# mitenjain/nanopore

Hardware: AMD Instinct MI355X
Metric: DP cells/sec (banded pair-HMM realign: forward + backward + posterior per cell) (higher is better)
Workload: dtype f32

## Files before the change

### nanopore_amd/csrc/npr_device.h

```cpp
#pragma once
#include <cstdint>

#include "npr_internal.h"
#include "npr_band.h"

namespace npr {

struct Task {
    int64_t x_off;
    int64_t y_off;
    int64_t band_off;
    int64_t pair_off;
    int32_t lX, lY;
    int32_t D;
    int32_t pair_cap;
    int32_t flags;
    int32_t model;
    int32_t xs, ys;
    int32_t read;
    int32_t cells_pad;
    int64_t ctl_off;
    int64_t tile_off;
    int64_t rowmask_off;
};

struct Stripe {
    int32_t X;
    int32_t K;
    int32_t df, dl;
    uint32_t row0;
    int32_t pad[3];
};

struct TaskOut {
    float tot_m;
    int32_t tot_e;
    float btot_m;
    int32_t btot_e;
    int32_t npairs;
    int32_t status;
};

struct KernelArgs {
    const Task *tasks;
    TaskOut *outs;
    int32_t *queue;
    int32_t ntasks;
    const DevModel *models;
    const uint8_t *seq;
    const int32_t *lo;
    const int32_t *n;
    const uint32_t *coff;
    const Stripe *stripes;
    const uint32_t *rowmask;
    unsigned long long *prof;
    const int64_t *region;
    const uint32_t *ctl;
    char *F;
    int64_t slot_stride;
    int32_t slot_base;
    int32_t *px;
    int32_t *py;
    float *pp;
    float threshold;
    int32_t wcap;
    float *Bv;
    int32_t *Be;
    float *ring;
    float *Fx;
    double *em_T;
    double *em_E;
};

constexpr int EM_BINS = 32;

struct CompactArgs {
    const Task *tasks;
    const TaskOut *outs;
    const int64_t *dst_off;
    int32_t ntasks;
    const int32_t *px;
    const int32_t *py;
    const float *pp;
    int32_t *cx;
    int32_t *cy;
    float *cp;
};

int launch_generic(const KernelArgs &a, int grid, int threads, size_t lds_bytes, bool dense, bool global_ring, void *stream);
int launch_em(const KernelArgs &a, int grid, size_t lds_bytes, bool global_ring, void *stream);
size_t em_extra_lds_bytes();
int launch_compact(const CompactArgs &a, void *stream);
int launch_stair(const KernelArgs &a, int R, int grid, void *stream);
int launch_wide(const KernelArgs &a, int R, int NW, int grid, void *stream);
int launch_em_stair(const KernelArgs &a, int R, int grid, void *stream);
size_t em_stair_lds_bytes();
struct MeaArgs {
    const Task *tasks;
    const TaskOut *outs;
    int32_t ntasks, n_reads;
    const int32_t *px, *py;
    const float *pp;
    const int64_t *rx_off;
    const int64_t *ry_off;
    const int64_t *rp_off;
    int32_t *cnt, *start, *colsum;
    int32_t *sx, *sy, *sq, *back;
    int32_t *kx, *ky, *kq, *kback;
    int4 *vrec;
    int32_t *kept;
    const int32_t *np, *poff, *pboff, *lane_read, *lane_piece;
    int32_t *pb, *pbest;
    int32_t n_pieces;
    int32_t *best_who;
    int32_t *read_flag;
    double gap_gamma, match_gamma;
    int32_t ring;
    const int32_t *order;
    const int32_t *read_first, *read_ntasks, *task_of;
    int32_t sort_lds_bytes;
    int32_t sort_threads;
    int32_t any_global_sort;
    const int64_t *cnt_off;
    int32_t ring_only;
    int32_t *ops_tmp;
    const int64_t *ot_off;
    int32_t *n_ops, *chain_len;
    int64_t *chain_mass;
    uint32_t *ops_dense;
    const int64_t *od_off;
    int32_t *max_run;
    uint16_t *ops_dense16;
};
int launch_tile(const KernelArgs &a, int R, int NW, int grid, void *stream, bool flat = false);
size_t tile_lds_bytes(int nw);
int64_t tile_scratch_cells(int64_t rows, int R);
struct PlanSeg {
    int64_t point_first;
    int64_t band_off;
    int32_t pieces, lX, lY, pad;
};
struct SegSummary {
    int64_t cells;
    int64_t generic_cells;
    int32_t max_width;
    int32_t bad;
    int32_t rough;
    int32_t pad;
};
constexpr int kSchedClasses = 7;
constexpr int kSchedR[kSchedClasses] = {1, 2, 4, 2, 2, 4, 4};
constexpr int kSchedNW[kSchedClasses] = {1, 1, 1, 4, 8, 8, 12};
struct PlanArgs {
    int32_t n_segs, fixed_mode, width;
    const PlanPoint *points;
    const PlanSeg *segs;
    int32_t *lo, *n;
    SegSummary *summary;
};
struct SchedArgs {
    int32_t n_segs;
    const PlanSeg *segs;
    const SegSummary *summary;
    const int32_t *lo, *n;
    const int64_t *ctl_off;
    const uint32_t *cand;
    uint32_t *ctl;
    int32_t *cls;
    int64_t *cells;
};
struct StripeArgs {
    int32_t count, R;
    const int32_t *seg_index;
    const PlanSeg *segs;
    const SegSummary *summary;
    const int32_t *lo, *n;
    const int64_t *tile_off;
    Stripe *stripes;
    int64_t *rows;
};
struct CoffArgs {
    int32_t n_segs;
    const PlanSeg *segs;
    const int32_t *n;
    uint32_t *coff;
};
int launch_plan_bands(const PlanArgs &a, void *stream);
template <int R>
NPR_HD constexpr uint32_t row_bias() { return R == 4 ? 2048u : 1024u; }
NPR_HD constexpr bool stair_fits(int64_t rows, int slots) { return rows * slots < (int64_t(1) << 29) - 512; }
struct RowMaskArgs {
    int32_t count;
    const int32_t *seg_index;
    const PlanSeg *segs;
    const int32_t *lo, *n;
    const int64_t *tile_off;
    const Stripe *stripes;
    const int64_t *mask_off;
    uint32_t *out;
};
int launch_plan_rowmask(const RowMaskArgs &a, void *stream);
size_t plan_sched_chunk_bytes(int64_t n_chunks);
int64_t plan_sched_chunks_of(int64_t D);
int launch_plan_sched(const SchedArgs &a, const int64_t *chunk_off, int64_t n_chunks, void *chunks, int32_t *cur, uint32_t cand_union, void *stream);
// ... 80 lines not shown
```

### nanopore_amd/csrc/npr_finish.cpp

```cpp
#include "npr_api_internal.h"

extern "C" {

}
namespace npr_impl {

int32_t fetch_pairs(npr_batch *b) {
    npr_ctx *ctx = b->ctx;
    if (b->pairs_ready) return NPR_OK;
    StageTimer tm("fetch_pairs");
    const int64_t ntasks = static_cast<int64_t>(b->tasks.size());
    const std::vector<int64_t> &dst = b->task_dst;
    const int32_t *hx = nullptr, *hy = nullptr;
    const float *hp = nullptr;
    const int64_t total = ntasks ? dst[ntasks] : 0;
    if (total) {
        DevBuf<int64_t> d_dst;
        DevBuf<int32_t> d_cx, d_cy;
        DevBuf<float> d_cp;
        hipError_t e;
        if ((e = d_dst.alloc_from(ctx, ntasks + 1)) != hipSuccess || (e = d_cx.alloc_from(ctx, total)) != hipSuccess ||
            (e = d_cy.alloc_from(ctx, total)) != hipSuccess || (e = d_cp.alloc_from(ctx, total)) != hipSuccess)
            return fail(ctx, NPR_ERR_NOMEM, "npr_batch_finish: hipMalloc", e);
        HIP_TRY(ctx, hipMemcpyAsync(d_dst.p, dst.data(), d_dst.bytes(), hipMemcpyHostToDevice, ctx->stream));
// ... 100 lines not shown
        if (b->read_status[i] != NPR_OK) return;
        int32_t *out = runs + 3 * run_off[i];
        int64_t x = 0, y = 0;
        for (int64_t q = b->guide_off[i]; q < b->guide_off[i + 1]; ++q) {
            const int32_t op = b->guide_ops[2 * q], len = b->guide_ops[2 * q + 1];
            if (op == NPR_OP_M) {
                if (len > 0) out[0] = static_cast<int32_t>(x), out[1] = static_cast<int32_t>(y), out[2] = len, out += 3;
                x += len, y += len;
            } else if (op == NPR_OP_I) {
                y += len;
            } else {
                x += len;
            }
        }
    });
    tm.lap("runs");
    DevBuf<int64_t> d_run_off;
    DevBuf<int32_t> d_runs;
    hipError_t e;
    if ((e = d_run_off.alloc_from(ctx, n + 1)) != hipSuccess || (e = b->d_rs_gx_off.alloc_from(ctx, n + 1)) != hipSuccess ||
        (e = d_runs.alloc_from(ctx, std::max<size_t>(3 * static_cast<size_t>(run_off[n]), 1))) != hipSuccess ||
        (e = b->d_rs_gy.alloc_from(ctx, std::max<int64_t>(gx_off[n], 1))) != hipSuccess)
        return fail(ctx, NPR_ERR_NOMEM, "npr_batch_create: hipMalloc (rescore tables)", e);
    HIP_TRY(ctx, hipMemcpyAsync(d_run_off.p, run_off.data(), sizeof(int64_t) * (n + 1), hipMemcpyHostToDevice, ctx->stream));
    HIP_TRY(ctx, hipMemcpyAsync(b->d_rs_gx_off.p, gx_off.data(), sizeof(int64_t) * (n + 1), hipMemcpyHostToDevice, ctx->stream));
    if (run_bytes) HIP_TRY(ctx, hipMemcpyAsync(d_runs.p, runs, run_bytes, hipMemcpyHostToDevice, ctx->stream));
    HIP_TRY(ctx, hipMemsetAsync(b->d_rs_gy.p, 0xff, sizeof(int32_t) * std::max<int64_t>(gx_off[n], 1), ctx->stream));
    RescoreArgs ra{static_cast<int32_t>(n), 0, d_run_off.p, d_runs.p, b->d_rs_gx_off.p, b->d_rs_gy.p, nullptr, nullptr, nullptr, nullptr, nullptr, nullptr, shift};
    const int rc = launch_rescore_table(ra, ctx->stream);
    if (rc != 0) return fail(ctx, NPR_ERR_HIP, "k_rescore_table launch", static_cast<hipError_t>(rc));
    HIP_TRY(ctx, hipStreamSynchronize(ctx->stream));
    tm.lap("table");
    b->rs_shift = shift, b->rs_staged = true;
    return NPR_OK;
}

int32_t rescore_sum(npr_batch *b, std::vector<double> &score) {
    npr_ctx *ctx = b->ctx;
    const int64_t n = b->n_reads, ntasks = static_cast<int64_t>(b->tasks.size());
    DevBuf<unsigned long long> d_sum;
    hipError_t e;
    if ((e = d_sum.alloc_from(ctx, n)) != hipSuccess) return fail(ctx, NPR_ERR_NOMEM, "npr_batch_finish: hipMalloc (rescore sums)", e);
    HIP_TRY(ctx, hipMemsetAsync(d_sum.p, 0, sizeof(unsigned long long) * n, ctx->stream));
    RescoreArgs ra{static_cast<int32_t>(n), static_cast<int32_t>(ntasks), nullptr, nullptr, b->d_rs_gx_off.p, b->d_rs_gy.p, b->d_tasks.p, b->d_outs.p,
                   b->d_px.p, b->d_py.p, b->d_pp.p, d_sum.p, b->rs_shift};
    const int rc = launch_rescore_sum(ra, ctx->stream);
    if (rc != 0) return fail(ctx, NPR_ERR_HIP, "k_rescore_sum launch", static_cast<hipError_t>(rc));
    std::vector<unsigned long long> sum(n);
    HIP_TRY(ctx, hipMemcpyAsync(sum.data(), d_sum.p, sizeof(unsigned long long) * n, hipMemcpyDeviceToHost, ctx->stream));
    HIP_TRY(ctx, hipStreamSynchronize(ctx->stream));
    score.assign(n, 0.0);
    for (int64_t i = 0; i < n; ++i)
        if (b->rs_columns[i] > 0) score[i] = std::ldexp(static_cast<double>(sum[i]), -b->rs_shift) / static_cast<double>(b->rs_columns[i]);
    return NPR_OK;
}

int32_t device_mea(npr_batch *b) {
    npr_ctx *ctx = b->ctx;
    std::unique_lock<std::mutex> arena_lock(ctx->arena->mu, std::defer_lock);
    if (!ctx->overlap) arena_lock.lock();
    ++ctx->arena->epoch;
    StageTimer tm("device_mea");
    const int64_t n = b->n_reads, ntasks = static_cast<int64_t>(b->tasks.size());
    std::vector<int64_t> rx(n + 1, 0), ry(n + 1, 0), rp(n + 1, 0), ot(n + 1, 0), od(n + 1, 0);
    for (int64_t i = 0; i < n; ++i) {
        const bool ok = b->results[i].status == NPR_OK;
        const int64_t lX = ok ? b->ref_len[i] : 0, lY = ok ? b->read_len[i] : 0, np = ok ? b->pair_off[i + 1] - b->pair_off[i] : 0;
        rx[i + 1] = rx[i] + lX + 1;
        ry[i + 1] = ry[i] + lY;
        rp[i + 1] = rp[i] + np;
        ot[i + 1] = ot[i] + 3 * std::min({np, lX, lY}) + 2;
    }
    const int ring = 8192;
    const int64_t total = rp[n];
    constexpr int64_t kMaxPieces = 64, kLanesWanted = 64 * 5 * 256;
    const int64_t kPiecePairs = std::min<int64_t>(2048, std::max<int64_t>(128, total / kLanesWanted));
    std::vector<int32_t> np(n);
    int64_t n_pieces = 0;
    for (int64_t i = 0; i < n; ++i) np[i] = static_cast<int32_t>(std::min(kMaxPieces, std::max<int64_t>(1, (rp[i + 1] - rp[i] + kPiecePairs - 1) / kPiecePairs))), n_pieces += np[i];
    if (!ctx->mea) ctx->mea = new MeaScratch;
    MeaScratch &m = *ctx->mea;
    hipError_t e;
    const int64_t lds_span = ctx->opt[NPR_OPT_MEA_GLOBAL_SORT] != 0 ? 0 : 16 * 1024;
    int64_t span = 0;
    std::vector<int64_t> cnt_off(n + 1, -1);
    int64_t cnt_total = 0;
    for (int64_t i = 0; i < n; ++i) {
        const int64_t sp = std::max(rx[i + 1] - rx[i], ry[i + 1] - ry[i]);
        if (sp <= lds_span) span = std::max(span, sp);
        else cnt_off[i] = cnt_total, cnt_total += rx[i + 1] - rx[i];
    }
    const bool sort_in_lds = cnt_total == 0;
    const size_t ntask_map = b->task_of.size();
    const size_t n_cnt = sort_in_lds ? 1 : static_cast<size_t>(cnt_total);
    {
        auto al = [](size_t bytes) { return (bytes + 255) & ~size_t(255); };
        const size_t need = al(8 * 5 * (n + 1)) + al(8 * n) + al(8 * (n + 1)) + 2 * al(4 * n_cnt) + al(4 * (ry[n] + 1)) + al(4 * (12 * total + 16)) +
                            al(4 * 6 * n) + al(4 * 2 * ot[n]) + al(4 * (3 * n + ntask_map)) + al(4 * ot[n]) + al(4 * (4 * n_pieces + 4 * n));
        const bool arena_fits = ctx->arena->F && need <= static_cast<size_t>(ctx->arena->cells.load()) * 8;
        bool in_arena = !ctx->overlap && arena_fits;
        for (;;) {
            char *cur = ctx->arena->F;
            if (in_arena && poison_byte() >= 0) {
                HIP_TRY(ctx, hipStreamSynchronize(ctx->stream));
                poison(ctx->arena->F, need);
            }
            auto take = [&](auto &buf, size_t count) -> hipError_t {
                using T = std::remove_pointer_t<decltype(buf.p)>;
                if (!in_arena) return buf.reserve(count);
                buf.borrow(reinterpret_cast<T *>(cur), count);
                cur += al(sizeof(T) * count);
                return hipSuccess;
            };
            if ((e = take(m.off, 5 * (n + 1))) == hipSuccess && (e = take(m.mass, n)) == hipSuccess && (e = take(m.od, n + 1)) == hipSuccess &&
                (e = take(m.cnt, n_cnt)) == hipSuccess && (e = take(m.start, n_cnt)) == hipSuccess && (e = take(m.col, ry[n] + 1)) == hipSuccess &&
                (e = take(m.sorted, 12 * total + 16)) == hipSuccess && (e = take(m.small, 6 * n)) == hipSuccess && (e = take(m.tmp, 2 * ot[n])) == hipSuccess &&
                (e = take(m.map, 3 * n + ntask_map)) == hipSuccess && (e = take(m.dense, ot[n])) == hipSuccess &&
                (e = take(m.pieces, 4 * n_pieces + 4 * n)) == hipSuccess)
                break;
            (void)hipGetLastError();
            if (!in_arena && ctx->overlap && arena_fits) {
                m.off.release(), m.mass.release(), m.od.release(), m.cnt.release(), m.start.release(), m.col.release(), m.sorted.release();
                m.small.release(), m.tmp.release(), m.map.release(), m.dense.release(), m.pieces.release();
                ctx->cache_flush();
                arena_lock.lock();
                if (!(ctx->arena->F && need <= static_cast<size_t>(ctx->arena->cells.load()) * 8)) return 1;
                ++ctx->arena->epoch;
                in_arena = true;
                continue;
            }
            return 1;
        }
    }
    HIP_TRY(ctx, hipMemcpyAsync(m.map.p, b->read_first_task.data(), sizeof(int32_t) * n, hipMemcpyHostToDevice, ctx->stream));
    HIP_TRY(ctx, hipMemcpyAsync(m.map.p + n, b->read_ntasks.data(), sizeof(int32_t) * n, hipMemcpyHostToDevice, ctx->stream));
    HIP_TRY(ctx, hipMemcpyAsync(m.map.p + 2 * n, b->task_of.data(), sizeof(int32_t) * ntask_map, hipMemcpyHostToDevice, ctx->stream));
    std::vector<int32_t> order(n);
    std::iota(order.begin(), order.end(), 0);
    std::stable_sort(order.begin(), order.end(), [&](int32_t x, int32_t y) { return rp[x + 1] - rp[x] > rp[y + 1] - rp[y]; });
    HIP_TRY(ctx, hipMemcpyAsync(m.map.p + 2 * n + ntask_map, order.data(), sizeof(int32_t) * n, hipMemcpyHostToDevice, ctx->stream));
    {
        std::vector<int32_t> tab(3 * n + 2 * n_pieces);
        int32_t *const t_np = tab.data(), *const t_poff = t_np + n, *const t_pboff = t_poff + n, *const t_lr = t_pboff + n, *const t_lp = t_lr + n_pieces;
        int64_t at = 0;
        for (int64_t k = 0; k < n; ++k) {
            const int32_t r = order[k];
            t_np[r] = np[r], t_poff[r] = static_cast<int32_t>(at), t_pboff[r] = static_cast<int32_t>(at + k);
            for (int32_t j = 0; j < np[r]; ++j) t_lr[at + j] = r, t_lp[at + j] = j;
            at += np[r];
        }
        HIP_TRY(ctx, hipMemcpyAsync(m.pieces.p, tab.data(), sizeof(int32_t) * tab.size(), hipMemcpyHostToDevice, ctx->stream));
    }
    std::vector<int64_t> offs(5 * (n + 1));
    std::copy(cnt_off.begin(), cnt_off.end(), offs.begin() + 4 * (n + 1));
    std::copy(rx.begin(), rx.end(), offs.begin());
    std::copy(ry.begin(), ry.end(), offs.begin() + (n + 1));
    std::copy(rp.begin(), rp.end(), offs.begin() + 2 * (n + 1));
    std::copy(ot.begin(), ot.end(), offs.begin() + 3 * (n + 1));
    HIP_TRY(ctx, hipMemcpyAsync(m.off.p, offs.data(), m.off.bytes(), hipMemcpyHostToDevice, ctx->stream));
    HIP_TRY(ctx, hipMemsetAsync(m.small.p, 0, m.small.bytes(), ctx->stream));
    MeaArgs a{};
    a.tasks = b->d_tasks.p, a.outs = b->d_outs.p, a.ntasks = static_cast<int32_t>(ntasks), a.n_reads = static_cast<int32_t>(n);
    a.px = b->d_px.p, a.py = b->d_py.p, a.pp = b->d_pp.p;
    a.rx_off = m.off.p, a.ry_off = m.off.p + (n + 1), a.rp_off = m.off.p + 2 * (n + 1), a.ot_off = m.off.p + 3 * (n + 1);
    a.cnt = m.cnt.p, a.start = m.start.p, a.colsum = m.col.p;
    a.sx = m.sorted.p, a.sy = m.sorted.p + total + 1, a.sq = m.sorted.p + 2 * (total + 1), a.back = m.sorted.p + 3 * (total + 1);
    a.kx = m.sorted.p + 4 * (total + 1), a.ky = m.sorted.p + 5 * (total + 1), a.kq = m.sorted.p + 6 * (total + 1), a.kback = m.sorted.p + 7 * (total + 1);
    a.vrec = reinterpret_cast<int4 *>(m.sorted.p + ((8 * (total + 1) + 3) & ~int64_t(3)));
    a.best_who = m.small.p, a.read_flag = m.small.p + n, a.n_ops = m.small.p + 2 * n, a.chain_len = m.small.p + 3 * n, a.kept = m.small.p + 4 * n, a.max_run = m.small.p + 5 * n;
    a.chain_mass = m.mass.p;
    a.np = m.pieces.p, a.poff = m.pieces.p + n, a.pboff = m.pieces.p + 2 * n, a.lane_read = m.pieces.p + 3 * n, a.lane_piece = m.pieces.p + 3 * n + n_pieces;
    a.pbest = m.pieces.p + 3 * n + 2 * n_pieces, a.pb = m.pieces.p + 3 * n + 3 * n_pieces, a.n_pieces = static_cast<int32_t>(n_pieces);
    a.gap_gamma = b->params.gap_gamma, a.match_gamma = b->params.match_gamma, a.ring = ring;
    a.ring_only = ctx->opt[NPR_OPT_MEA_RING_ONLY] != 0 ? 1 : 0;
    a.read_first = m.map.p, a.read_ntasks = m.map.p + n, a.task_of = m.map.p + 2 * n, a.order = m.map.p + 2 * n + ntask_map;
    a.sort_lds_bytes = static_cast<int32_t>(4 * span);
    a.sort_threads = ctx->overlap == 1 ? 512 : 0;
    a.any_global_sort = sort_in_lds ? 0 : 1;
    a.cnt_off = m.off.p + 4 * (n + 1);
    a.ops_tmp = m.tmp.p, a.od_off = m.od.p;
    int rc = launch_mea_sort(a, ctx->stream);
    if (rc == 0) rc = launch_mea_chain(a, ctx->stream);
    if (rc != 0) return fail(ctx, NPR_ERR_HIP, "MEA kernel launch", static_cast<hipError_t>(rc));
    std::vector<int32_t> small(6 * n);
    std::vector<int64_t> mass(n);
    HIP_TRY(ctx, hipMemcpyAsync(small.data(), m.small.p, m.small.bytes(), hipMemcpyDeviceToHost, ctx->stream));
    HIP_TRY(ctx, hipMemcpyAsync(mass.data(), m.mass.p, m.mass.bytes(), hipMemcpyDeviceToHost, ctx->stream));
    HIP_TRY(ctx, hipStreamSynchronize(ctx->stream));
    tm.lap("sort + chain + trace");
    const int32_t *flag = small.data() + n, *nops = small.data() + 2 * n, *clen = small.data() + 3 * n;
    int32_t longest = 0;
    for (int64_t i = 0; i < n; ++i)
        if (b->results[i].status == NPR_OK && flag[i] == NPR_ERR_CAPACITY) return 1;
    for (int64_t i = 0; i < n; ++i) {
        npr_read_result &r = b->results[i];
        if (r.status == NPR_OK && flag[i] != 0) r.status = flag[i];
        const int64_t k = r.status == NPR_OK ? nops[i] : 0;
        od[i + 1] = od[i] + k;
        if (k) longest = std::max(longest, small[5 * n + i]);
        r.n_ops = k;
        r.score = (r.status == NPR_OK && clen[i] > 0) ? static_cast<double>(mass[i]) / (static_cast<double>(clen[i]) * PROB_ONE) : 0.0;
    }
    b->ops_off = od;
    b->ops_words = 2 * od[n];
    b->have_pairs_form = false, b->have_packed_form = true;
    if (od[n] > b->packed_cap)
        for (size_t i = 0; i < ctx->packed_pool.size(); ++i)
            if (ctx->packed_pool[i].cap >= od[n]) {
                b->packed = std::move(ctx->packed_pool[i].p), b->packed_cap = ctx->packed_pool[i].cap;
                ctx->packed_pool.erase(ctx->packed_pool.begin() + static_cast<std::ptrdiff_t>(i));
                break;
            }
    if (od[n] > b->packed_cap) {
        b->packed.reset(new uint32_t[od[n] + od[n] / 8]);
        b->packed_cap = od[n] + od[n] / 8;
    }
    if (od[n]) {
        const bool narrow = longest < (1 << 14) && ctx->opt[NPR_OPT_MEA_WIDE_OPS] == 0 &&
                            sizeof(uint16_t) * static_cast<size_t>(od[n]) <= m.sorted.bytes();
        a.ops_dense = m.dense.p;
        a.ops_dense16 = narrow ? reinterpret_cast<uint16_t *>(m.sorted.p) : nullptr;
        HIP_TRY(ctx, hipMemcpyAsync(m.od.p, od.data(), m.od.bytes(), hipMemcpyHostToDevice, ctx->stream));
        if ((rc = launch_mea_gather(a, ctx->stream)) != 0) return fail(ctx, NPR_ERR_HIP, "k_mea_gather launch", static_cast<hipError_t>(rc));
        const size_t word = narrow ? sizeof(uint16_t) : sizeof(uint32_t), need = word * static_cast<size_t>(od[n]);
        if (need > ctx->pin_pairs_bytes) {
            if (ctx->pin_pairs) (void)hipHostFree(ctx->pin_pairs);
            ctx->pin_pairs = nullptr, ctx->pin_pairs_bytes = 0;
            if ((e = hipHostMalloc(&ctx->pin_pairs, need + need / 4, hipHostMallocDefault)) != hipSuccess)
                return fail(ctx, NPR_ERR_NOMEM, "npr_batch_finish: hipHostMalloc", e);
            ctx->pin_pairs_bytes = need + need / 4;
        }
        constexpr int64_t kOpsPieces = 48;
        const int64_t nops_all = od[n], pieces = std::min<int64_t>(kOpsPieces, (nops_all + (1 << 20) - 1) >> 20);
        const int64_t piece = ((nops_all + pieces - 1) / pieces + 63) & ~int64_t(63);
        while (static_cast<int64_t>(ctx->ops_events.size()) < pieces) {
            hipEvent_t ev;
            if ((e = hipEventCreateWithFlags(&ev, hipEventDisableTiming)) != hipSuccess) return fail(ctx, NPR_ERR_HIP, "hipEventCreate", e);
            ctx->ops_events.push_back(ev);
        }
        const char *dev = narrow ? reinterpret_cast<const char *>(a.ops_dense16) : reinterpret_cast<const char *>(m.dense.p);
        char *pin = static_cast<char *>(ctx->pin_pairs);
        for (int64_t c = 0; c < pieces; ++c) {
            const int64_t lo = std::min(nops_all, c * piece), hi = std::min(nops_all, lo + piece);
            if (hi > lo) HIP_TRY(ctx, hipMemcpyAsync(pin + word * lo, dev + word * lo, word * static_cast<size_t>(hi - lo), hipMemcpyDeviceToHost, ctx->stream));
            HIP_TRY(ctx, hipEventRecord(ctx->ops_events[c], ctx->stream));
        }
        uint32_t *out = b->packed.get();
        std::atomic<int> failed{0};
        parallel_for(pieces, ctx->host_threads, [&](int64_t c) {
            if (hipSetDevice(ctx->device) != hipSuccess || hipEventSynchronize(ctx->ops_events[c]) != hipSuccess) {
                failed = 1;
                return;
            }
            const int64_t lo = std::min(nops_all, c * piece), hi = std::min(nops_all, lo + piece);
            if (narrow) {
                const uint16_t *src = reinterpret_cast<const uint16_t *>(pin);
                for (int64_t i = lo; i < hi; ++i) out[i] = src[i];
            } else {
                std::memcpy(out + lo, pin + word * lo, word * static_cast<size_t>(hi - lo));
// ... 279 lines not shown
```

### nanopore_amd/csrc/npr_mea.hip

```cpp
#include <hip/hip_runtime.h>

#include "npr_device.h"

namespace npr {
namespace {

constexpr int64_t P1 = PROB_ONE;
constexpr int WAVE = 64;
constexpr int SORT_THREADS = 1024;

__device__ __forceinline__ int rdlane(int v, int j) { return __builtin_amdgcn_readlane(v, j); }
__device__ __forceinline__ int64_t rdlane64(int64_t v, int j) {
    const int lo = __builtin_amdgcn_readlane(static_cast<int>(v), j);
    const int hi = __builtin_amdgcn_readlane(static_cast<int>(v >> 32), j);
    return (static_cast<int64_t>(hi) << 32) | static_cast<uint32_t>(lo);
}
__device__ __forceinline__ void wave_sync() {
    __builtin_amdgcn_fence(__ATOMIC_RELEASE, "wavefront");
    __builtin_amdgcn_wave_barrier();
    __builtin_amdgcn_fence(__ATOMIC_ACQUIRE, "wavefront");
}
__device__ __forceinline__ bool beats(int64_t s, int w, int64_t os, int ow) { return s > os || (s == os && w > ow); }

__device__ __forceinline__ int mea_task_pairs(const TaskOut &o, const Task &tk) { return o.status == NPR_OK ? min(max(o.npairs, 0), tk.pair_cap) : 0; }
__device__ __forceinline__ bool mea_is_posterior(float p) { return p >= 0.f && p <= 1.0f + 0x1p-10f; }

__global__ void __launch_bounds__(256) k_mea_zero(MeaArgs a) {
    const int r = blockIdx.x;
    const int64_t c0 = a.cnt_off[r];
    if (c0 < 0) return;
    const int nx = static_cast<int>(a.rx_off[r + 1] - a.rx_off[r]), ny = static_cast<int>(a.ry_off[r + 1] - a.ry_off[r]);
    for (int i = threadIdx.x; i < nx; i += blockDim.x) a.cnt[c0 + i] = 0;
    for (int i = threadIdx.x; i < ny; i += blockDim.x) a.colsum[a.ry_off[r] + i] = 0;
}

__global__ void __launch_bounds__(256) k_mea_count(MeaArgs a) {
    for (int t = blockIdx.x; t < a.ntasks; t += gridDim.x) {
        const Task &tk = a.tasks[t];
        const int n = mea_task_pairs(a.outs[t], tk);
        const int r = tk.read;
        const int64_t rx = a.cnt_off[r], ry = a.ry_off[r];
        if (rx < 0) continue;
        const int lX = static_cast<int>(a.rx_off[r + 1] - a.rx_off[r]) - 1, lY = static_cast<int>(a.ry_off[r + 1] - ry);
        for (int i = threadIdx.x; i < n; i += blockDim.x) {
            const int x = a.px[tk.pair_off + i], y = a.py[tk.pair_off + i];
            if (x < 0 || x >= lX || y < 0 || y >= lY || !mea_is_posterior(a.pp[tk.pair_off + i])) {
                a.read_flag[r] = NPR_ERR_INVALID;
                continue;
            }
            const int q = static_cast<int>(floor(static_cast<double>(a.pp[tk.pair_off + i]) * static_cast<double>(P1)));
            atomicAdd(a.cnt + rx + x, 1);
            atomicAdd(a.colsum + ry + y, q);
        }
    }
}

__global__ void __launch_bounds__(256) k_mea_scan(MeaArgs a) {
    __shared__ int wsum[4];
    const int r = blockIdx.x, tid = threadIdx.x, lane = tid & 63, wv = tid >> 6;
    const int64_t rx = a.cnt_off[r];
    if (rx < 0) return;
    const int n = static_cast<int>(a.rx_off[r + 1] - a.rx_off[r]);
    int carry = 0;
    for (int base = 0; base < n; base += 256) {
        const int i = base + tid;
        const int v = i < n ? a.cnt[rx + i] : 0;
        int s = v;
        for (int o = 1; o < WAVE; o <<= 1) {
            const int t = __shfl_up(s, o);
            if (lane >= o) s += t;
        }
        if (lane == WAVE - 1) wsum[wv] = s;
        __syncthreads();
        int before = 0, total = 0;
        for (int k = 0; k < 4; ++k) before += k < wv ? wsum[k] : 0, total += wsum[k];
        if (i < n) a.start[rx + i] = carry + before + s - v;
        carry += total;
        __syncthreads();
    }
}

__global__ void __launch_bounds__(256) k_mea_scatter(MeaArgs a) {
    for (int t = blockIdx.x; t < a.ntasks; t += gridDim.x) {
        const Task &tk = a.tasks[t];
        const int n = mea_task_pairs(a.outs[t], tk);
        const int r = tk.read;
        const int64_t rx = a.cnt_off[r], rp = a.rp_off[r];
        if (rx < 0) continue;
        const int lX = static_cast<int>(a.rx_off[r + 1] - a.rx_off[r]) - 1, lY = static_cast<int>(a.ry_off[r + 1] - a.ry_off[r]);
        for (int i = threadIdx.x; i < n; i += blockDim.x) {
            const int x = a.px[tk.pair_off + i], y = a.py[tk.pair_off + i];
            if (x < 0 || x >= lX || y < 0 || y >= lY || !mea_is_posterior(a.pp[tk.pair_off + i])) continue;
            const int q = static_cast<int>(floor(static_cast<double>(a.pp[tk.pair_off + i]) * static_cast<double>(P1)));
            const int64_t pos = rp + a.start[rx + x] + (atomicSub(a.cnt + rx + x, 1) - 1);
            a.sx[pos] = x, a.sy[pos] = y, a.sq[pos] = q;
        }
    }
}

__global__ void __launch_bounds__(SORT_THREADS) k_mea_sort_lds(MeaArgs a) {
    extern __shared__ int h[];
    __shared__ int wsum[SORT_THREADS / WAVE];
    const int r = a.order[blockIdx.x], tid = threadIdx.x, lane = tid & 63, wv = tid >> 6;
    const int nthreads = static_cast<int>(blockDim.x);
    const int64_t rx = a.rx_off[r], ry = a.ry_off[r], rp = a.rp_off[r];
    const int lX = static_cast<int>(a.rx_off[r + 1] - rx) - 1, lY = static_cast<int>(a.ry_off[r + 1] - ry);
    if (a.rp_off[r + 1] == rp || a.cnt_off[r] >= 0) return;
    const int ft = a.read_first[r], nt = a.read_ntasks[r];
    int bad = 0;
    auto for_pairs = [&](auto f) {
        for (int s = 0; s < nt; ++s) {
            const int t = a.task_of[ft + s];
            const Task &tk = a.tasks[t];
            const int n = mea_task_pairs(a.outs[t], tk);
            for (int i = tid; i < n; i += nthreads) {
                const int x = a.px[tk.pair_off + i], y = a.py[tk.pair_off + i];
                if (x < 0 || x >= lX || y < 0 || y >= lY || !mea_is_posterior(a.pp[tk.pair_off + i])) {
                    bad = 1;
                    continue;
                }
                f(x, y, static_cast<int>(floor(static_cast<double>(a.pp[tk.pair_off + i]) * static_cast<double>(P1))));
            }
        }
    };
    for (int i = tid; i < lY; i += nthreads) h[i] = 0;
    __syncthreads();
    for_pairs([&](int, int y, int q) { atomicAdd(&h[y], q); });
    __syncthreads();
    for (int i = tid; i < lY; i += nthreads) a.colsum[ry + i] = h[i];
    __syncthreads();
    for (int i = tid; i <= lX; i += nthreads) h[i] = 0;
    __syncthreads();
    for_pairs([&](int x, int, int) { atomicAdd(&h[x], 1); });
    __syncthreads();
    int carry = 0;
    for (int base = 0; base <= lX; base += nthreads) {
        const int i = base + tid;
        const int v = i <= lX ? h[i] : 0;
        int sc = v;
        for (int o = 1; o < WAVE; o <<= 1) {
            const int t = __shfl_up(sc, o);
            if (lane >= o) sc += t;
        }
        if (lane == WAVE - 1) wsum[wv] = sc;
        __syncthreads();
        int before = 0, total = 0;
        for (int k = 0; k < nthreads / WAVE; ++k) before += k < wv ? wsum[k] : 0, total += wsum[k];
        if (i <= lX) h[i] = carry + before + sc - v;
        carry += total;
        __syncthreads();
    }
    for_pairs([&](int x, int y, int q) {
        const int64_t pos = rp + atomicAdd(&h[x], 1);
        a.sx[pos] = x, a.sy[pos] = y, a.sq[pos] = q;
    });
    if (bad) a.read_flag[r] = NPR_ERR_INVALID;
}

constexpr int MEA_RETRY = 1;

struct Chunk {
    int valid;
    uint64_t ends;
    uint64_t keep;
    int y, q;
    int64_t w;
    int who;
};
__device__ __forceinline__ Chunk prep_chunk(const MeaArgs &a, int *sx, int *sy, int *sq, int64_t ry, int base, int n, int lane,
                                            int64_t floor_w, int64_t *tw, int *ty, int *tq) {
    Chunk c;
    const int pos = base + lane;
    const bool in = pos < n;
    const int x = in ? sx[pos] : -1, xn = pos + 1 < n ? sx[pos + 1] : -2;
    int y = in ? sy[pos] : 0, q = in ? sq[pos] : 0;
    const uint64_t ends = __ballot(in && x != xn);
    c.valid = ends ? 64 - __builtin_clzll(ends) : 0;
    c.ends = ends, c.keep = 0, c.y = 0, c.q = 0, c.w = 0;
    if (!ends) return c;
    const bool act = lane < c.valid;
    const uint64_t starts = (ends << 1) | 1ull;
    const int gfirst = 63 - __builtin_clzll(starts & (lane == 63 ? ~0ull : ((2ull << lane) - 1)));
    const int gend = act ? lane + __builtin_ctzll(ends >> lane) : lane;
    const int gsize = gend - gfirst + 1;
    int rank = 0, rowsum = q;
    for (int o = 1; __any(act && o < gsize); ++o) {
        const int lo = lane - o, hi = lane + o;
        const int yl = __shfl(y, lo & 63), ql = __shfl(q, lo & 63), yh = __shfl(y, hi & 63), qh = __shfl(q, hi & 63);
        if (lo >= gfirst) rank += yl < y ? 1 : 0, rowsum += ql;
        if (hi <= gend) rank += yh < y ? 1 : 0, rowsum += qh;
    }
    const int colsum = act ? a.colsum[ry + y] : 0;
    const int64_t gap = max(P1 - rowsum, int64_t(0)) + max(P1 - colsum, int64_t(0));
    const int64_t w0 = q - static_cast<int64_t>(floor(a.gap_gamma * static_cast<double>(gap)));
    wave_sync();
    if (act) {
        const int to = gend - rank;
        tw[to] = w0, ty[to] = y, tq[to] = q;
    }
    wave_sync();
    c.w = tw[lane], c.y = ty[lane], c.q = tq[lane];
    c.keep = __ballot(act && c.w > floor_w);
    c.who = gfirst + gend - lane;
    if (act) sy[base + c.who] = c.y, sq[base + c.who] = c.q;
    return c;
}

constexpr int WEIGH_CHUNK = 128;
constexpr int WEIGH_RING = 512;
constexpr int WEIGH_HALO = 64;
__device__ __forceinline__ int64_t pair_weight(int q, int rowsum, int colsum, double gap_gamma) {
    const int64_t gap = max(P1 - rowsum, int64_t(0)) + max(P1 - colsum, int64_t(0));
    return q - static_cast<int64_t>(floor(gap_gamma * static_cast<double>(gap)));
}
__global__ void __launch_bounds__(WAVE) k_mea_weigh(MeaArgs a) {
    __shared__ int X[WEIGH_RING], Y[WEIGH_RING], Q[WEIGH_RING], C[WEIGH_RING];
    const int r = a.order[blockIdx.x], lane = threadIdx.x;
    const int64_t rp = a.rp_off[r], ry = a.ry_off[r];
    const int n = a.read_flag[r] ? 0 : static_cast<int>(a.rp_off[r + 1] - rp);
    const int *const sx = a.sx + rp, *const sy = a.sy + rp, *const sq = a.sq + rp;
    const int *const col = a.colsum + ry;
    const int64_t floor_w = static_cast<int64_t>(floor(a.match_gamma * static_cast<double>(P1)));
    constexpr int RM = WEIGH_RING - 1;
    const int nc = (n + WEIGH_CHUNK - 1) / WEIGH_CHUNK;
    int giveup = 0;
    int fx[2], fy[2], fq[2];
    auto fetch = [&](int chunk) {
#pragma unroll
        for (int h = 0; h < 2; ++h) {
            const int j = chunk * WEIGH_CHUNK + h * WAVE + lane;
            const bool ok = j < n;
            fx[h] = ok ? sx[j] : -1, fy[h] = ok ? sy[j] : 0, fq[h] = ok ? sq[j] : 0;
        }
    };
    auto stage = [&](int chunk) {
        int fc[2];
#pragma unroll
        for (int h = 0; h < 2; ++h) fc[h] = fx[h] >= 0 ? col[fy[h]] : 0;
#pragma unroll
        for (int h = 0; h < 2; ++h) {
            const int k = (chunk * WEIGH_CHUNK + h * WAVE + lane) & RM;
            X[k] = fx[h], Y[k] = fy[h], Q[k] = fq[h], C[k] = fc[h];
        }
    };
    for (int k = lane; k < WEIGH_CHUNK; k += WAVE) X[(-WEIGH_CHUNK + k) & RM] = -2;
    if (nc > 0) {
        fetch(0);
        stage(0);
        fetch(1);
    }
    int carry = 0;
    for (int c = 0; c < nc; ++c) {
        stage(c + 1);
        fetch(c + 2);
        wave_sync();
        int keep[2], below[2], above[2], before[2], xs[2], ys[2], qs[2];
        int64_t ws[2];
#pragma unroll
        for (int h = 0; h < 2; ++h) {
            const int i = c * WEIGH_CHUNK + h * WAVE + lane, me = i & RM;
            const bool in = i < n;
            const int x = X[me], y = Y[me], q = Q[me];
            int gs = i, ge = i, rowsum = q;
            if (in) {
                while (gs > i - WEIGH_HALO && X[(gs - 1) & RM] == x) rowsum += Q[(--gs) & RM];
                while (ge < i + WEIGH_HALO && X[(ge + 1) & RM] == x) rowsum += Q[(++ge) & RM];
                if (gs == i - WEIGH_HALO || ge == i + WEIGH_HALO) giveup = 1;
            }
            const int64_t w = in ? pair_weight(q, rowsum, C[me], a.gap_gamma) : 0;
            keep[h] = in && w > floor_w;
            before[h] = below[h] = above[h] = 0;
            if (keep[h])
                for (int j = gs; j <= ge; ++j) {
                    const int k = j & RM;
                    if (j != i && pair_weight(Q[k], rowsum, C[k], a.gap_gamma) > floor_w) before[h] += j < i, below[h] += Y[k] < y, above[h] += Y[k] > y;
                }
            xs[h] = x, ys[h] = y, qs[h] = q, ws[h] = w;
        }
        int sc0 = keep[0], sc1 = keep[1];
        for (int o = 1; o < WAVE; o <<= 1) {
            const int t0 = __shfl_up(sc0, o), t1 = __shfl_up(sc1, o);
            if (lane >= o) sc0 += t0, sc1 += t1;
        }
        const int tot0 = __shfl(sc0, WAVE - 1), tot1 = __shfl(sc1, WAVE - 1);
        const int ex[2] = {sc0 - keep[0], tot0 + sc1 - keep[1]};
#pragma unroll
        for (int h = 0; h < 2; ++h)
            if (keep[h]) {
                const int64_t g0 = rp + carry + ex[h] - before[h];
                const int64_t id = g0 + below[h], at = g0 + above[h];
                a.kx[id] = xs[h], a.ky[id] = ys[h], a.kq[id] = qs[h];
                a.vrec[at] = make_int4(ys[h], static_cast<int>(ws[h]), static_cast<int>(id - rp), 0);
            }
        carry += tot0 + tot1;
        wave_sync();
    }
    giveup = __any(giveup);
    if (lane == 0) {
        a.kept[r] = giveup ? -1 : carry;
        if (giveup && a.read_flag[r] == 0) a.read_flag[r] = MEA_RETRY;
// ... 251 lines not shown
        if (len <= 0) return;
        if (op == hop) {
            hlen += len;
            return;
        }
        if (hop >= 0 && p > lo) {
            --p;
            if (lane == 0) *p = make_int2(hop, hlen);
            longest = max(longest, hlen);
        }
        hop = op, hlen = len;
    };
    int cx = lX, cy = lY, len = 0;
    int64_t mass = 0;
    bool broken = false;
    const bool alive = a.read_flag[r] == 0;
    int piece = by_id ? __builtin_amdgcn_readfirstlane(a.np[r]) : 1;
    const int *const pbest = a.pbest + (by_id ? a.poff[r] : 0);
    while (piece-- > 0) {
    int i = !alive ? -1 : __builtin_amdgcn_readfirstlane(by_id ? pbest[piece] : a.best_who[r]);
    while (i >= 0) {
        const int cb = max(i - (WAVE - 1), 0), idx = min(cb + lane, i);
        const int vb = back[idx], vx = sx[idx], vy = sy[idx], vq = sq[idx];
        const int rel = (vb - cb) & (WAVE - 1);
        const bool diag = vb >= cb && __shfl(vx, rel) == vx - 1 && __shfl(vy, rel) == vy - 1;
        int nxt = diag ? rel : lane, val = diag ? vq : 0;
#pragma unroll
        for (int k = 0; k < 6; ++k) {
            val += __shfl(val, nxt);
            nxt = __shfl(nxt, nxt);
        }
        while (i >= cb) {
            const int l = i - cb, h = rdlane(nxt, l);
            const int x = rdlane(vx, l), y = rdlane(vy, l), hx = rdlane(vx, h), hy = rdlane(vy, h);
            emit(NPR_OP_I, cy - y - 1);
            emit(NPR_OP_D, cx - x - 1);
            emit(NPR_OP_M, x - hx + 1);
            cx = hx, cy = hy, mass += rdlane(val, l) + rdlane(vq, h), len += x - hx + 1;
            const int to = rdlane(vb, h);
            if (to >= i) {
                broken = true;
                i = -1;
                break;
            }
            i = to;
        }
    }
    if (broken) break;
    }
    emit(NPR_OP_I, cy);
    emit(NPR_OP_D, cx);
    if (hop >= 0 && p > lo) {
        --p;
        if (lane == 0) *p = make_int2(hop, hlen);
        longest = max(longest, hlen);
    }
    if (lane == 0) {
        if (broken) a.read_flag[r] = NPR_ERR_INVALID;
        a.max_run[r] = longest;
        a.n_ops[r] = broken ? 0 : static_cast<int>(reinterpret_cast<int2 *>(a.ops_tmp) + a.ot_off[r + 1] - p);
        a.chain_len[r] = len;
        a.chain_mass[r] = mass;
    }
}

__global__ void __launch_bounds__(256) k_mea_gather(MeaArgs a) {
    for (int r = blockIdx.x; r < a.n_reads; r += gridDim.x) {
        const int n = static_cast<int>(a.od_off[r + 1] - a.od_off[r]);
        const int2 *src = reinterpret_cast<const int2 *>(a.ops_tmp) + a.ot_off[r + 1] - a.n_ops[r];
        uint32_t *dst = a.ops_dense + a.od_off[r];
        uint16_t *const dst16 = a.ops_dense16 ? a.ops_dense16 + a.od_off[r] : nullptr;
        for (int i = threadIdx.x; i < n; i += blockDim.x) {
            const uint32_t w = static_cast<uint32_t>(src[i].y) << 2 | static_cast<uint32_t>(src[i].x);
            dst[i] = w;
            if (dst16) dst16[i] = static_cast<uint16_t>(w);
        }
    }
}

}

size_t mea_chain_lds_bytes(int ring) { return static_cast<size_t>(ring) * 12 + WAVE * (8 + 4 + 4); }

int launch_mea_sort(const MeaArgs &a, void *stream) {
    hipStream_t s = static_cast<hipStream_t>(stream);
    if (a.sort_lds_bytes > 0) {
        const hipError_t e = hipFuncSetAttribute(reinterpret_cast<const void *>(k_mea_sort_lds), hipFuncAttributeMaxDynamicSharedMemorySize, a.sort_lds_bytes);
        if (e != hipSuccess) return static_cast<int>(e);
        hipLaunchKernelGGL(k_mea_sort_lds, dim3(a.n_reads), dim3(a.sort_threads >= WAVE && a.sort_threads < SORT_THREADS ? a.sort_threads & ~(WAVE - 1) : SORT_THREADS), a.sort_lds_bytes, s, a);
    }
    if (a.any_global_sort) {
        const int tg = a.ntasks < 8192 ? (a.ntasks > 0 ? a.ntasks : 1) : 8192;
        hipLaunchKernelGGL(k_mea_zero, dim3(a.n_reads), dim3(256), 0, s, a);
        hipLaunchKernelGGL(k_mea_count, dim3(tg), dim3(256), 0, s, a);
        hipLaunchKernelGGL(k_mea_scan, dim3(a.n_reads), dim3(256), 0, s, a);
        hipLaunchKernelGGL(k_mea_scatter, dim3(tg), dim3(256), 0, s, a);
    }
    return static_cast<int>(hipGetLastError());
}

int launch_mea_chain(const MeaArgs &a, void *stream) {
    hipStream_t s = static_cast<hipStream_t>(stream);
    const size_t lds = mea_chain_lds_bytes(a.ring);
    const hipError_t e = hipFuncSetAttribute(reinterpret_cast<const void *>(k_mea_chain), hipFuncAttributeMaxDynamicSharedMemorySize, static_cast<int>(lds));
    if (e != hipSuccess) return static_cast<int>(e);
    const int lanes_lds = LWIN * WAVE * static_cast<int>(sizeof(int64_t));
    const hipError_t e2 = hipFuncSetAttribute(reinterpret_cast<const void *>(k_mea_chain_lanes), hipFuncAttributeMaxDynamicSharedMemorySize, lanes_lds);
    if (e2 != hipSuccess) return static_cast<int>(e2);
    hipLaunchKernelGGL(k_mea_weigh, dim3(a.n_reads), dim3(WAVE), 0, s, a);
    hipLaunchKernelGGL(k_mea_cuts, dim3(a.n_reads), dim3(WAVE), 0, s, a);
    hipLaunchKernelGGL(k_mea_chain_lanes, dim3((a.n_pieces + WAVE - 1) / WAVE), dim3(WAVE), lanes_lds, s, a);
    hipLaunchKernelGGL(k_mea_chain, dim3(a.n_reads < 512 ? (a.n_reads > 0 ? a.n_reads : 1) : 512), dim3(WAVE), lds, s, a);
    hipLaunchKernelGGL(k_mea_trace, dim3(a.n_reads), dim3(WAVE), 0, s, a);
    return static_cast<int>(hipGetLastError());
}

int launch_mea_gather(const MeaArgs &a, void *stream) {
    const int g = a.n_reads < 8192 ? a.n_reads : 8192;
    hipLaunchKernelGGL(k_mea_gather, dim3(g), dim3(256), 0, static_cast<hipStream_t>(stream), a);
    return static_cast<int>(hipGetLastError());
}

}
```

Before: 372.0 billion.

## Fuse MEA sort and weigh into one LDS front kernel for small reads

Adds a k_mea_front kernel that, for reads with fewer than 65536 pairs and a small span, does a counting sort by x using 16-bit packed LDS counters, computes row and column sums, and filters and ranks kept pairs inline. It replaces the separate LDS sort and weigh passes for those reads, cutting global traffic and launches. Reads flagged for retry are re-sorted later by a new resort kernel before chaining. The cost is more complex code, and the per-x rank computation is quadratic in group size.

```diff
diff --git a/nanopore_amd/csrc/npr_device.h b/nanopore_amd/csrc/npr_device.h
--- a/nanopore_amd/csrc/npr_device.h
+++ b/nanopore_amd/csrc/npr_device.h
@@ -95,6 +95,8 @@
 int launch_wide(const KernelArgs &a, int R, int NW, int grid, void *stream);
 int launch_em_stair(const KernelArgs &a, int R, int grid, void *stream);
 size_t em_stair_lds_bytes();
+constexpr int64_t MEA_SORT_LDS = -1;
+constexpr int64_t MEA_FRONT = -2;
 struct MeaArgs {
     const Task *tasks;
     const TaskOut *outs;
@@ -119,7 +121,9 @@
     const int32_t *order;
     const int32_t *read_first, *read_ntasks, *task_of;
     int32_t sort_lds_bytes;
+    int32_t front_lds_bytes;
     int32_t sort_threads;
+    int32_t any_sort_lds;
     int32_t any_global_sort;
     const int64_t *cnt_off;
     int32_t ring_only;
diff --git a/nanopore_amd/csrc/npr_finish.cpp b/nanopore_amd/csrc/npr_finish.cpp
--- a/nanopore_amd/csrc/npr_finish.cpp
+++ b/nanopore_amd/csrc/npr_finish.cpp
@@ -206,13 +206,19 @@
     MeaScratch &m = *ctx->mea;
     hipError_t e;
     const int64_t lds_span = ctx->opt[NPR_OPT_MEA_GLOBAL_SORT] != 0 ? 0 : 16 * 1024;
-    int64_t span = 0;
-    std::vector<int64_t> cnt_off(n + 1, -1);
+    int64_t span = 0, front_bytes = 0;
+    std::vector<int64_t> cnt_off(n + 1, MEA_SORT_LDS);
     int64_t cnt_total = 0;
+    bool any_sort_lds = false;
     for (int64_t i = 0; i < n; ++i) {
         const int64_t sp = std::max(rx[i + 1] - rx[i], ry[i + 1] - ry[i]);
-        if (sp <= lds_span) span = std::max(span, sp);
-        else cnt_off[i] = cnt_total, cnt_total += rx[i + 1] - rx[i];
+        if (sp <= lds_span) {
+            span = std::max(span, sp);
+            if (rp[i + 1] - rp[i] < (int64_t(1) << 16)) cnt_off[i] = MEA_FRONT, front_bytes = std::max(front_bytes, 4 * (ry[i + 1] - ry[i]) + 4 * ((rx[i + 1] - rx[i] + 1) / 2));
+            else any_sort_lds = true;
+        } else {
+            cnt_off[i] = cnt_total, cnt_total += rx[i + 1] - rx[i];
+        }
     }
     const bool sort_in_lds = cnt_total == 0;
     const size_t ntask_map = b->task_of.size();
@@ -299,6 +305,8 @@
     a.ring_only = ctx->opt[NPR_OPT_MEA_RING_ONLY] != 0 ? 1 : 0;
     a.read_first = m.map.p, a.read_ntasks = m.map.p + n, a.task_of = m.map.p + 2 * n, a.order = m.map.p + 2 * n + ntask_map;
     a.sort_lds_bytes = static_cast<int32_t>(4 * span);
+    a.front_lds_bytes = static_cast<int32_t>(front_bytes);
+    a.any_sort_lds = any_sort_lds ? 1 : 0;
     a.sort_threads = ctx->overlap == 1 ? 512 : 0;
     a.any_global_sort = sort_in_lds ? 0 : 1;
     a.cnt_off = m.off.p + 4 * (n + 1);
diff --git a/nanopore_amd/csrc/npr_mea.hip b/nanopore_amd/csrc/npr_mea.hip
--- a/nanopore_amd/csrc/npr_mea.hip
+++ b/nanopore_amd/csrc/npr_mea.hip
@@ -98,14 +98,11 @@
     }
 }
 
-__global__ void __launch_bounds__(SORT_THREADS) k_mea_sort_lds(MeaArgs a) {
-    extern __shared__ int h[];
-    __shared__ int wsum[SORT_THREADS / WAVE];
-    const int r = a.order[blockIdx.x], tid = threadIdx.x, lane = tid & 63, wv = tid >> 6;
+__device__ void sort_read_lds(const MeaArgs &a, int r, int *h, int *wsum) {
+    const int tid = threadIdx.x, lane = tid & 63, wv = tid >> 6;
     const int nthreads = static_cast<int>(blockDim.x);
     const int64_t rx = a.rx_off[r], ry = a.ry_off[r], rp = a.rp_off[r];
     const int lX = static_cast<int>(a.rx_off[r + 1] - rx) - 1, lY = static_cast<int>(a.ry_off[r + 1] - ry);
-    if (a.rp_off[r + 1] == rp || a.cnt_off[r] >= 0) return;
     const int ft = a.read_first[r], nt = a.read_ntasks[r];
     int bad = 0;
     auto for_pairs = [&](auto f) {
@@ -157,7 +154,196 @@
     if (bad) a.read_flag[r] = NPR_ERR_INVALID;
 }
 
+__global__ void __launch_bounds__(SORT_THREADS) k_mea_sort_lds(MeaArgs a) {
+    extern __shared__ int h[];
+    __shared__ int wsum[SORT_THREADS / WAVE];
+    const int r = a.order[blockIdx.x];
+    if (a.rp_off[r + 1] == a.rp_off[r] || a.cnt_off[r] != MEA_SORT_LDS) return;
+    sort_read_lds(a, r, h, wsum);
+}
+
 constexpr int MEA_RETRY = 1;
+
+__global__ void __launch_bounds__(SORT_THREADS) k_mea_resort(MeaArgs a) {
+    extern __shared__ int h[];
+    __shared__ int wsum[SORT_THREADS / WAVE];
+    for (int r = blockIdx.x; r < a.n_reads; r += gridDim.x) {
+        if (a.read_flag[r] != MEA_RETRY || a.cnt_off[r] != MEA_FRONT) continue;
+        __syncthreads();
+        sort_read_lds(a, r, h, wsum);
+    }
+}
+
+__device__ __forceinline__ int64_t pair_weight(int q, int rowsum, int colsum, double gap_gamma) {
+    const int64_t gap = max(P1 - rowsum, int64_t(0)) + max(P1 - colsum, int64_t(0));
+    return q - static_cast<int64_t>(floor(gap_gamma * static_cast<double>(gap)));
+}
+
+__device__ __forceinline__ void lds_barrier() {
+    __builtin_amdgcn_fence(__ATOMIC_RELEASE, "workgroup", "local");
+    __builtin_amdgcn_s_barrier();
+    __builtin_amdgcn_fence(__ATOMIC_ACQUIRE, "workgroup", "local");
+}
+
+__device__ __forceinline__ int block_exclusive_sum(int v, int *wsum, int &total) {
+    const int tid = threadIdx.x, lane = tid & 63, wv = tid >> 6, nw = static_cast<int>(blockDim.x) / WAVE;
+    int sc = v;
+    for (int o = 1; o < WAVE; o <<= 1) {
+        const int t = __shfl_up(sc, o);
+        if (lane >= o) sc += t;
+    }
+    if (lane == WAVE - 1) wsum[wv] = sc;
+    lds_barrier();
+    int before = 0;
+    total = 0;
+    for (int k = 0; k < nw; ++k) before += k < wv ? wsum[k] : 0, total += wsum[k];
+    lds_barrier();
+    return before + sc - v;
+}
+
+constexpr int FRONT_REG = 8;
+__global__ void __launch_bounds__(SORT_THREADS) k_mea_front(MeaArgs a) {
+    extern __shared__ int lds_front[];
+    __shared__ int wsum[SORT_THREADS / WAVE];
+    const int r = a.order[blockIdx.x], tid = threadIdx.x;
+    if (a.cnt_off[r] != MEA_FRONT) return;
+    const int nthreads = static_cast<int>(blockDim.x);
+    const int64_t rx = a.rx_off[r], ry = a.ry_off[r], rp = a.rp_off[r];
+    const int lX = static_cast<int>(a.rx_off[r + 1] - rx) - 1, lY = static_cast<int>(a.ry_off[r + 1] - ry);
+    const int n = static_cast<int>(a.rp_off[r + 1] - rp);
+    if (n == 0) return;
+    int *const C = lds_front;
+    unsigned *const Ew = reinterpret_cast<unsigned *>(C + lY);
+    unsigned short *const E = reinterpret_cast<unsigned short *>(Ew);
+    const int ft = a.read_first[r], nt = a.read_ntasks[r];
+    int bad = 0;
+    auto for_pairs = [&](auto f) {
+        for (int s = 0; s < nt; ++s) {
+            const int t = a.task_of[ft + s];
+            const Task &tk = a.tasks[t];
+            const int np = mea_task_pairs(a.outs[t], tk);
+            for (int i = tid; i < np; i += nthreads) {
+                const int x = a.px[tk.pair_off + i], y = a.py[tk.pair_off + i];
+                const float p = a.pp[tk.pair_off + i];
+                if (x < 0 || x >= lX || y < 0 || y >= lY || !mea_is_posterior(p)) {
+                    bad = 1;
+                    continue;
+                }
+                f(x, y, static_cast<int>(floor(static_cast<double>(p) * static_cast<double>(P1))));
+            }
+        }
+    };
+    const int ew = (lX + 2) >> 1;
+    for (int i = tid; i < lY; i += nthreads) C[i] = 0;
+    for (int i = tid; i < ew; i += nthreads) Ew[i] = 0;
+    __syncthreads();
+    for_pairs([&](int x, int y, int q) {
+        atomicAdd(&C[y], q);
+        atomicAdd(&Ew[x >> 1], 1u << ((x & 1) << 4));
+    });
+    if (__syncthreads_or(bad)) {
+        if (tid == 0) a.read_flag[r] = NPR_ERR_INVALID;
+        return;
+    }
+    {
+        const int per = (lX + nthreads) / nthreads, i0 = min(tid * per, lX + 1), i1 = min(i0 + per, lX + 1);
+        int v = 0;
+        for (int i = i0; i < i1; ++i) v += E[i];
+        int total;
+        int run = block_exclusive_sum(v, wsum, total);
+        for (int i = i0; i < i1; ++i) {
+            const int c = E[i];
+            E[i] = static_cast<unsigned short>(run);
+            run += c;
+        }
+    }
+    __syncthreads();
+    int *const sy = a.sy + rp, *const sq = a.sq + rp;
+    for_pairs([&](int x, int y, int q) {
+        const int sh = (x & 1) << 4;
+        const int pos = static_cast<int>((atomicAdd(&Ew[x >> 1], 1u << sh) >> sh) & 0xffffu);
+        sy[pos] = y, sq[pos] = q;
+    });
+    __syncthreads();
+    const int64_t floor_w = static_cast<int64_t>(floor(a.match_gamma * static_cast<double>(P1)));
+    const double gg = a.gap_gamma;
+    int *const kx = a.kx + rp, *const ky = a.ky + rp, *const kq = a.kq + rp;
+    int4 *const vrec = a.vrec + rp;
+    int kept = 0;
+    auto wave_max = [](int v) {
+        for (int o = 32; o; o >>= 1) v = max(v, __shfl_xor(v, o));
+        return __builtin_amdgcn_readfirstlane(v);
+    };
+    int ngs, nge, ngm, nys[FRONT_REG], nqs[FRONT_REG];
+    auto fetch = [&](int x) {
+        ngs = x < lX && x > 0 ? E[x - 1] : 0, nge = x < lX ? E[x] : 0;
+        const int g = nge - ngs <= FRONT_REG ? nge - ngs : 0;
+        ngm = wave_max(g);
+#pragma unroll
+        for (int u = 0; u < FRONT_REG; ++u)
+            if (u < ngm) nys[u] = u < g ? sy[ngs + u] : 0, nqs[u] = u < g ? sq[ngs + u] : 0;
+    };
+    fetch(tid);
+    for (int base = 0; base < lX; base += nthreads) {
+        const int x = base + tid;
+        const int gs = ngs, ge = nge, gm = ngm;
+        const bool small = ge - gs <= FRONT_REG;
+        int ys[FRONT_REG], qs[FRONT_REG];
+        int ws[FRONT_REG];
+        unsigned kp = 0;
+#pragma unroll
+        for (int u = 0; u < FRONT_REG; ++u)
+            if (u < gm) ys[u] = nys[u], qs[u] = nqs[u];
+        fetch(x + nthreads);
+        int rowsum = 0, k = 0;
+        if (small) {
+#pragma unroll
+            for (int u = 0; u < FRONT_REG; ++u)
+                if (u < gm && gs + u < ge) rowsum += qs[u];
+#pragma unroll
+            for (int u = 0; u < FRONT_REG; ++u)
+                if (u < gm && gs + u < ge) {
+                    const int64_t w = pair_weight(qs[u], rowsum, C[ys[u]], gg);
+                    ws[u] = static_cast<int>(w);
+                    if (w > floor_w) kp |= 1u << u, ++k;
+                }
+        } else {
+            for (int j = gs; j < ge; ++j) rowsum += sq[j];
+            for (int j = gs; j < ge; ++j) k += pair_weight(sq[j], rowsum, C[sy[j]], gg) > floor_w;
+        }
+        int total;
+        const int g0 = kept + block_exclusive_sum(k, wsum, total);
+        if (k && small) {
+#pragma unroll
+            for (int u = 0; u < FRONT_REG; ++u)
+                if (u < gm && ((kp >> u) & 1)) {
+                    int rank = 0;
+#pragma unroll
+                    for (int v = 0; v < FRONT_REG; ++v)
+                        if (v < gm) rank += v != u && ((kp >> v) & 1) && (ys[v] < ys[u] || (ys[v] == ys[u] && (qs[v] < qs[u] || (qs[v] == qs[u] && v < u))));
+                    const int id = g0 + rank;
+                    kx[id] = x, ky[id] = ys[u], kq[id] = qs[u];
+                    vrec[g0 + k - 1 - rank] = make_int4(ys[u], ws[u], id, 0);
+                }
+        } else if (k) {
+            for (int j = gs; j < ge; ++j) {
+                const int y = sy[j], q = sq[j];
+                const int64_t w = pair_weight(q, rowsum, C[y], gg);
+                if (w <= floor_w) continue;
+                int rank = 0;
+                for (int i = gs; i < ge; ++i) {
+                    const int yi = sy[i], qi = sq[i];
+                    if (i != j && (yi < y || (yi == y && (qi < q || (qi == q && i < j)))) && pair_weight(qi, rowsum, C[yi], gg) > floor_w) ++rank;
+                }
+                const int id = g0 + rank;
+                kx[id] = x, ky[id] = y, kq[id] = q;
+                vrec[g0 + k - 1 - rank] = make_int4(y, static_cast<int>(w), id, 0);
+            }
+        }
+        kept += total;
+    }
+    if (tid == 0) a.kept[r] = kept;
+}
 
 struct Chunk {
     int valid;
@@ -209,13 +395,10 @@
 constexpr int WEIGH_CHUNK = 128;
 constexpr int WEIGH_RING = 512;
 constexpr int WEIGH_HALO = 64;
-__device__ __forceinline__ int64_t pair_weight(int q, int rowsum, int colsum, double gap_gamma) {
-    const int64_t gap = max(P1 - rowsum, int64_t(0)) + max(P1 - colsum, int64_t(0));
-    return q - static_cast<int64_t>(floor(gap_gamma * static_cast<double>(gap)));
-}
 __global__ void __launch_bounds__(WAVE) k_mea_weigh(MeaArgs a) {
     __shared__ int X[WEIGH_RING], Y[WEIGH_RING], Q[WEIGH_RING], C[WEIGH_RING];
     const int r = a.order[blockIdx.x], lane = threadIdx.x;
+    if (a.cnt_off[r] == MEA_FRONT) return;
     const int64_t rp = a.rp_off[r], ry = a.ry_off[r];
     const int n = a.read_flag[r] ? 0 : static_cast<int>(a.rp_off[r + 1] - rp);
     const int *const sx = a.sx + rp, *const sy = a.sy + rp, *const sq = a.sq + rp;
@@ -633,12 +816,21 @@
 
 size_t mea_chain_lds_bytes(int ring) { return static_cast<size_t>(ring) * 12 + WAVE * (8 + 4 + 4); }
 
+static int sort_block(const MeaArgs &a) { return a.sort_threads >= WAVE && a.sort_threads < SORT_THREADS ? a.sort_threads & ~(WAVE - 1) : SORT_THREADS; }
+
 int launch_mea_sort(const MeaArgs &a, void *stream) {
     hipStream_t s = static_cast<hipStream_t>(stream);
+    if (a.front_lds_bytes > 0) {
+        const hipError_t e = hipFuncSetAttribute(reinterpret_cast<const void *>(k_mea_front), hipFuncAttributeMaxDynamicSharedMemorySize, a.front_lds_bytes);
+        if (e != hipSuccess) return static_cast<int>(e);
+        hipLaunchKernelGGL(k_mea_front, dim3(a.n_reads), dim3(sort_block(a)), a.front_lds_bytes, s, a);
+    }
     if (a.sort_lds_bytes > 0) {
         const hipError_t e = hipFuncSetAttribute(reinterpret_cast<const void *>(k_mea_sort_lds), hipFuncAttributeMaxDynamicSharedMemorySize, a.sort_lds_bytes);
         if (e != hipSuccess) return static_cast<int>(e);
-        hipLaunchKernelGGL(k_mea_sort_lds, dim3(a.n_reads), dim3(a.sort_threads >= WAVE && a.sort_threads < SORT_THREADS ? a.sort_threads & ~(WAVE - 1) : SORT_THREADS), a.sort_lds_bytes, s, a);
+        const hipError_t e2 = hipFuncSetAttribute(reinterpret_cast<const void *>(k_mea_resort), hipFuncAttributeMaxDynamicSharedMemorySize, a.sort_lds_bytes);
+        if (e2 != hipSuccess) return static_cast<int>(e2);
+        if (a.any_sort_lds) hipLaunchKernelGGL(k_mea_sort_lds, dim3(a.n_reads), dim3(sort_block(a)), a.sort_lds_bytes, s, a);
     }
     if (a.any_global_sort) {
         const int tg = a.ntasks < 8192 ? (a.ntasks > 0 ? a.ntasks : 1) : 8192;
@@ -658,10 +850,12 @@
     const int lanes_lds = LWIN * WAVE * static_cast<int>(sizeof(int64_t));
     const hipError_t e2 = hipFuncSetAttribute(reinterpret_cast<const void *>(k_mea_chain_lanes), hipFuncAttributeMaxDynamicSharedMemorySize, lanes_lds);
     if (e2 != hipSuccess) return static_cast<int>(e2);
-    hipLaunchKernelGGL(k_mea_weigh, dim3(a.n_reads), dim3(WAVE), 0, s, a);
+    if (a.any_sort_lds || a.any_global_sort) hipLaunchKernelGGL(k_mea_weigh, dim3(a.n_reads), dim3(WAVE), 0, s, a);
     hipLaunchKernelGGL(k_mea_cuts, dim3(a.n_reads), dim3(WAVE), 0, s, a);
     hipLaunchKernelGGL(k_mea_chain_lanes, dim3((a.n_pieces + WAVE - 1) / WAVE), dim3(WAVE), lanes_lds, s, a);
-    hipLaunchKernelGGL(k_mea_chain, dim3(a.n_reads < 512 ? (a.n_reads > 0 ? a.n_reads : 1) : 512), dim3(WAVE), lds, s, a);
+    if (a.front_lds_bytes > 0)
+        hipLaunchKernelGGL(k_mea_resort, dim3(a.n_reads < 256 ? a.n_reads : 256), dim3(sort_block(a)), a.sort_lds_bytes, s, a);
+    hipLaunchKernelGGL(k_mea_chain,dim3(a.n_reads < 512 ? (a.n_reads > 0 ? a.n_reads : 1) : 512), dim3(WAVE), lds, s, a);
     hipLaunchKernelGGL(k_mea_trace, dim3(a.n_reads), dim3(WAVE), 0, s, a);
     return static_cast<int>(hipGetLastError());
 }
```

After: 371.5 billion (median of 2 runs). No clear change (-0.1%).
